# G-U-N/Phased-Consistency-Model

Measured on NVIDIA H100. Metric: distillation steps/sec (SD1.5 PCM-LoRA, bs=8/GPU), higher is better.
Workload: dtype bf16

## Files before the change

### pcm_b200/csrc/attn_wg.cu

```cuda
#include "common.cuh"
#include "wgmma.cuh"
#include "host_common.h"

namespace pcm {

namespace {

constexpr int kAwThreads = 384;
constexpr int kAwStages = 2;
constexpr int kTile = 64 * 128;

struct alignas(64) AttnWgParams {
  CUtensorMap q_map, k_map, v_map;
  bf16* out;
  float* lse;
  int H, Sq, Skv, D;
  long long ldo;
  float c;
};

template <int KB>
__global__ void __launch_bounds__(kAwThreads, 1) attn_fwd_wg_kernel(const __grid_constant__ AttnWgParams p) {
  extern __shared__ uint8_t smem_raw[];
  uint8_t* smem = reinterpret_cast<uint8_t*>((reinterpret_cast<uintptr_t>(smem_raw) + 1023) &
                                             ~static_cast<uintptr_t>(1023));
  uint8_t* sQ = smem;
  uint8_t* sK = sQ + 2 * KB * kTile;
  uint8_t* sV = sK + kAwStages * KB * kTile;
  __shared__ __align__(8) uint64_t q_bar;
  __shared__ __align__(8) uint64_t full_bar[kAwStages];
  __shared__ __align__(8) uint64_t empty_bar[kAwStages];

  const int wg = threadIdx.x >> 7;
  const int b = blockIdx.z, h = blockIdx.y, q0 = blockIdx.x * 128;
  const int nblk = (p.Skv + 63) / 64;
  constexpr uint32_t kv_bytes = 2 * KB * kTile;

  if (threadIdx.x == 0) {
    tma_prefetch_desc(&p.q_map);
    tma_prefetch_desc(&p.k_map);
    tma_prefetch_desc(&p.v_map);
    mbar_init(&q_bar, 1);
    for (int i = 0; i < kAwStages; ++i) {
      mbar_init(&full_bar[i], 1);
      mbar_init(&empty_bar[i], 2);
    }
    fence_barrier_init();
  }
  __syncthreads();
  griddep_sync();

  if (wg == 0) {
    if (threadIdx.x == 0) {
      mbar_arrive_expect_tx(&q_bar, 2 * KB * kTile);
      for (int w = 0; w < 2; ++w)
        for (int kb = 0; kb < KB; ++kb)
          tma_load_3d(sQ + (w * KB + kb) * kTile, &p.q_map, &q_bar, h * p.D + kb * 64, q0 + 64 * w, b);
      for (int j = 0; j < nblk; ++j) {
        const int st = j % kAwStages;
        mbar_wait(&empty_bar[st], ((j / kAwStages) & 1) ^ 1);
        mbar_arrive_expect_tx(&full_bar[st], kv_bytes);
        for (int kb = 0; kb < KB; ++kb) {
          tma_load_3d(sK + (st * KB + kb) * kTile, &p.k_map, &full_bar[st], h * p.D + kb * 64, j * 64, b);
          tma_load_3d(sV + (st * KB + kb) * kTile, &p.v_map, &full_bar[st], h * p.D + kb * 64, j * 64, b);
        }
      }
    }
    return;
  }

  const int cw = wg - 1, et = threadIdx.x & 127, warp = et >> 5, lane = et & 31;
  uint8_t* myQ = sQ + cw * KB * kTile;
  mbar_wait(&q_bar, 0);
  if (p.D < KB * 64) {
    const int c0 = p.D >> 3, nch = KB * 8;
    for (int i = et; i < 64 * nch; i += 128) {
      const int row = i / nch, ch = i - row * nch;
      if (ch < c0) continue;
      const uint32_t a = smem_u32(myQ + (ch >> 3) * kTile) + row * 128 + (((ch & 7) ^ (row & 7)) << 4);
      sts128(a, 0u, 0u, 0u, 0u);
    }
    fence_proxy_async();
  }
  asm volatile("bar.sync %0, 128;" ::"r"(1 + cw) : "memory");

  float o[KB][32];
#pragma unroll
  for (int kb = 0; kb < KB; ++kb)
#pragma unroll
    for (int i = 0; i < 32; ++i) o[kb][i] = 0.f;
  float m_run[2] = {-INFINITY, -INFINITY}, l_run[2] = {0.f, 0.f};
  const uint32_t q_addr = smem_u32(myQ);

  for (int j = 0; j < nblk; ++j) {
    const int st = j % kAwStages;
    mbar_wait(&full_bar[st], (j / kAwStages) & 1);
    const uint32_t k_addr = smem_u32(sK + st * KB * kTile);
    const uint32_t v_addr = smem_u32(sV + st * KB * kTile);
    float s[32];
    wgmma_fence();
#pragma unroll
    for (int kb = 0; kb < KB; ++kb)
#pragma unroll
      for (int k = 0; k < 4; ++k)
        Wgmma<64, 0, 0>::mma(s, wgmma_desc_sw128(q_addr + kb * kTile + k * 32, 16, 1024),
                             wgmma_desc_sw128(k_addr + kb * kTile + k * 32, 16, 1024), (kb | k) != 0 ? 1u : 0u);
    wgmma_commit();
    wgmma_wait<0>();
    wgmma_fence_acc(s);

    const int kbase = j * 64 + 2 * (lane & 3);
    float mx[2] = {-INFINITY, -INFINITY};
#pragma unroll
    for (int i = 0; i < 32; ++i) {
      const int key = kbase + 8 * (i >> 2) + (i & 1);
      const float v = key < p.Skv ? s[i] * p.c : -INFINITY;
      s[i] = v;
      mx[(i >> 1) & 1] = fmaxf(mx[(i >> 1) & 1], v);
    }
    float alpha[2];
#pragma unroll
    for (int r = 0; r < 2; ++r) {
      mx[r] = fmaxf(mx[r], __shfl_xor_sync(0xffffffffu, mx[r], 1));
      mx[r] = fmaxf(mx[r], __shfl_xor_sync(0xffffffffu, mx[r], 2));
      const float mn = fmaxf(m_run[r], mx[r]);
      alpha[r] = exp2f(m_run[r] - mn);
      m_run[r] = mn;
    }
    float rs[2] = {0.f, 0.f};
    uint32_t pa[4][4];
#pragma unroll
    for (int i = 0; i < 32; i += 2) {
      const int r = (i >> 1) & 1;
      const float p0 = exp2f(s[i] - m_run[r]), p1 = exp2f(s[i + 1] - m_run[r]);
      rs[r] += p0 + p1;
      pa[i >> 3][(i & 7) >> 1] = pack_bf16x2(p0, p1);
    }
#pragma unroll
    for (int r = 0; r < 2; ++r) l_run[r] = l_run[r] * alpha[r] + rs[r];
#pragma unroll
    for (int kb = 0; kb < KB; ++kb)
#pragma unroll
      for (int i = 0; i < 32; ++i) o[kb][i] *= alpha[(i >> 1) & 1];

    wgmma_fence();
#pragma unroll
    for (int kk = 0; kk < 4; ++kk)
#pragma unroll
      for (int kb = 0; kb < KB; ++kb)
        wgmma_rs_m64n64<1>(o[kb], pa[kk], wgmma_desc_sw128(v_addr + kb * kTile + kk * 2048, kTile, 1024), 1u);
    wgmma_commit();
    wgmma_wait<0>();
#pragma unroll
    for (int kb = 0; kb < KB; ++kb) wgmma_fence_acc(o[kb]);
    __syncwarp();
    if (et == 0) mbar_arrive(&empty_bar[st]);
  }

#pragma unroll
  for (int r = 0; r < 2; ++r) {
    l_run[r] += __shfl_xor_sync(0xffffffffu, l_run[r], 1);
    l_run[r] += __shfl_xor_sync(0xffffffffu, l_run[r], 2);
  }
  const int row0 = q0 + 64 * cw + 16 * warp + (lane >> 2);
#pragma unroll
  for (int r = 0; r < 2; ++r) {
    const int row = row0 + 8 * r;
    if (row >= p.Sq) continue;
    const float inv = 1.f / l_run[r];
    bf16* orow = p.out + (static_cast<long long>(b) * p.Sq + row) * p.ldo + h * p.D;
#pragma unroll
    for (int kb = 0; kb < KB; ++kb)
#pragma unroll
      for (int q = 0; q < 8; ++q) {
        const int col = kb * 64 + 8 * q + 2 * (lane & 3);
        if (col < p.D)
          *reinterpret_cast<uint32_t*>(orow + col) =
              pack_bf16x2(o[kb][4 * q + 2 * r] * inv, o[kb][4 * q + 2 * r + 1] * inv);
      }
    if ((lane & 3) == 0 && p.lse) p.lse[(static_cast<long long>(b) * p.H + h) * p.Sq + row] = m_run[r] + log2f(l_run[r]);
  }
}

struct alignas(64) AttnBwdParams {
  CUtensorMap fix0_map, fix1_map;
  CUtensorMap str0_map, str1_map;
  const float *lse, *delta;
  bf16 *out0, *out1;
  long long ld0, ld1;
  int H, Sq, Skv, D;
  int n_fix, n_str;
  float c, scale;
};

template <bool KV>
__global__ void __launch_bounds__(kAwThreads, 1) attn_bwd_wg_kernel(const __grid_constant__ AttnBwdParams p) {
  extern __shared__ uint8_t smem_raw[];
  uint8_t* smem = reinterpret_cast<uint8_t*>((reinterpret_cast<uintptr_t>(smem_raw) + 1023) &
                                             ~static_cast<uintptr_t>(1023));
  uint8_t* sF = smem;
  uint8_t* sS = sF + 4 * kTile;
  __shared__ __align__(8) uint64_t f_bar;
  __shared__ __align__(8) uint64_t full_bar[kAwStages];
  __shared__ __align__(8) uint64_t empty_bar[kAwStages];

  const int wg = threadIdx.x >> 7;
  const int b = blockIdx.z, h = blockIdx.y, r0 = blockIdx.x * 128;
  const int nblk = (p.n_str + 63) / 64;
  const int col0 = h * p.D;

  if (threadIdx.x == 0) {
    tma_prefetch_desc(&p.fix0_map);
    tma_prefetch_desc(&p.fix1_map);
    tma_prefetch_desc(&p.str0_map);
    tma_prefetch_desc(&p.str1_map);
    mbar_init(&f_bar, 1);
    for (int i = 0; i < kAwStages; ++i) {
      mbar_init(&full_bar[i], 1);
      mbar_init(&empty_bar[i], 2);
    }
    fence_barrier_init();
  }
  __syncthreads();
  griddep_sync();

  if (wg == 0) {
    regs_dealloc<40>();
    if (threadIdx.x == 0) {
      mbar_arrive_expect_tx(&f_bar, 4 * kTile);
      for (int w = 0; w < 2; ++w) {
        tma_load_3d(sF + (2 * w) * kTile, &p.fix0_map, &f_bar, col0, r0 + 64 * w, b);
        tma_load_3d(sF + (2 * w + 1) * kTile, &p.fix1_map, &f_bar, col0, r0 + 64 * w, b);
      }
      for (int j = 0; j < nblk; ++j) {
        const int st = j % kAwStages;
        mbar_wait(&empty_bar[st], ((j / kAwStages) & 1) ^ 1);
        mbar_arrive_expect_tx(&full_bar[st], 2 * kTile);
        tma_load_3d(sS + (2 * st) * kTile, &p.str0_map, &full_bar[st], col0, j * 64, b);
        tma_load_3d(sS + (2 * st + 1) * kTile, &p.str1_map, &full_bar[st], col0, j * 64, b);
      }
    }
    return;
  }

  regs_alloc<232>();
  const int cw = wg - 1, et = threadIdx.x & 127, warp = et >> 5, lane = et & 31;
  uint8_t* myF = sF + 2 * cw * kTile;
  mbar_wait(&f_bar, 0);
  if (p.D < 64) {
    const int c0 = p.D >> 3;
    for (int i = et; i < 2 * 64 * 8; i += 128) {
      const int t = i >> 9, row = (i >> 3) & 63, ch = i & 7;
      if (ch < c0) continue;
      sts128(smem_u32(myF + t * kTile) + row * 128 + ((ch ^ (row & 7)) << 4), 0u, 0u, 0u, 0u);
    }
    fence_proxy_async();
  }
  asm volatile("bar.sync %0, 128;" ::"r"(1 + cw) : "memory");

  const float* L = p.lse + (static_cast<long long>(b) * p.H + h) * p.Sq;
  const float* Dl = p.delta + (static_cast<long long>(b) * p.H + h) * p.Sq;
  const int frow = r0 + 64 * cw + 16 * warp + (lane >> 2);
  float lrow[2] = {0.f, 0.f}, drow[2] = {0.f, 0.f};
  bool rvalid[2];
#pragma unroll
  for (int r = 0; r < 2; ++r) {
    rvalid[r] = frow + 8 * r < p.n_fix;
    if (!KV) {
      lrow[r] = rvalid[r] ? L[frow + 8 * r] : INFINITY;
      drow[r] = rvalid[r] ? Dl[frow + 8 * r] : 0.f;
    }
  }
  float acc0[32], acc1[32];
#pragma unroll
  for (int i = 0; i < 32; ++i) acc0[i] = acc1[i] = 0.f;
  const uint32_t f0 = smem_u32(myF), f1 = f0 + kTile;

  for (int j = 0; j < nblk; ++j) {
    const int st = j % kAwStages;
    mbar_wait(&full_bar[st], (j / kAwStages) & 1);
    const uint32_t s0 = smem_u32(sS + 2 * st * kTile), s1 = s0 + kTile;
    float s[32], dp[32];
    wgmma_fence();
#pragma unroll
    for (int k = 0; k < 4; ++k) {
      Wgmma<64, 0, 0>::mma(s, wgmma_desc_sw128(f0 + k * 32, 16, 1024), wgmma_desc_sw128(s0 + k * 32, 16, 1024),
                           k != 0 ? 1u : 0u);
      Wgmma<64, 0, 0>::mma(dp, wgmma_desc_sw128(f1 + k * 32, 16, 1024), wgmma_desc_sw128(s1 + k * 32, 16, 1024),
                           k != 0 ? 1u : 0u);
    }
    wgmma_commit();
    float lc[16], dc[16];
    if (KV) {
#pragma unroll
      for (int q = 0; q < 8; ++q)
#pragma unroll
        for (int e = 0; e < 2; ++e) {
          const int qi = j * 64 + 8 * q + 2 * (lane & 3) + e;
          lc[2 * q + e] = qi < p.Sq ? L[qi] : INFINITY;
          dc[2 * q + e] = qi < p.Sq ? Dl[qi] : 0.f;
        }
    }
    wgmma_wait<0>();
    wgmma_fence_acc(s);
    wgmma_fence_acc(dp);
    uint32_t pa[4][4], dsa[4][4];
#pragma unroll
    for (int i = 0; i < 32; i += 2) {
      const int r = (i >> 1) & 1;
      float pv[2], g[2];
#pragma unroll
      for (int e = 0; e < 2; ++e) {
        const int col = 8 * (i >> 2) + 2 * (lane & 3) + e;
        float l, d;
        bool ok;
        if (KV) {
          l = lc[2 * (i >> 2) + e];
          d = dc[2 * (i >> 2) + e];
          ok = rvalid[r];
        } else {
          l = lrow[r];
          d = drow[r];
          ok = j * 64 + col < p.Skv;
        }
        pv[e] = ok ? exp2f(s[i + e] * p.c - l) : 0.f;
        g[e] = pv[e] * (dp[i + e] - d);
      }
      pa[i >> 3][(i & 7) >> 1] = pack_bf16x2(pv[0], pv[1]);
      dsa[i >> 3][(i & 7) >> 1] = pack_bf16x2(g[0], g[1]);
    }
    wgmma_fence();
#pragma unroll
    for (int kk = 0; kk < 4; ++kk) {
      wgmma_rs_m64n64<1>(acc0, dsa[kk], wgmma_desc_sw128(s0 + kk * 2048, kTile, 1024), 1u);
      if (KV) wgmma_rs_m64n64<1>(acc1, pa[kk], wgmma_desc_sw128(s1 + kk * 2048, kTile, 1024), 1u);
    }
    wgmma_commit();
    wgmma_wait<0>();
    wgmma_fence_acc(acc0);
    wgmma_fence_acc(acc1);
    __syncwarp();
    if (et == 0) mbar_arrive(&empty_bar[st]);
  }

#pragma unroll
  for (int r = 0; r < 2; ++r) {
    if (!rvalid[r]) continue;
    const long long row = static_cast<long long>(b) * p.n_fix + frow + 8 * r;
    bf16* o0 = p.out0 + row * p.ld0 + col0;
    bf16* o1 = KV ? p.out1 + row * p.ld1 + col0 : nullptr;
#pragma unroll
    for (int q = 0; q < 8; ++q) {
      const int col = 8 * q + 2 * (lane & 3);
      if (col < p.D) {
        *reinterpret_cast<uint32_t*>(o0 + col) =
            pack_bf16x2(acc0[4 * q + 2 * r] * p.scale, acc0[4 * q + 2 * r + 1] * p.scale);
        if (KV) *reinterpret_cast<uint32_t*>(o1 + col) = pack_bf16x2(acc1[4 * q + 2 * r], acc1[4 * q + 2 * r + 1]);
      }
    }
  }
}

int encode_seq_map(CUtensorMap* m, const void* base, int HD, int S, int B, long long ld) {
  if ((reinterpret_cast<uintptr_t>(base) & 15) != 0 || (ld & 7) != 0)
    return set_error("attention: tensor map base not 16-byte aligned or row stride not a multiple of 8");
  cuuint64_t dims[3] = {static_cast<cuuint64_t>(HD), static_cast<cuuint64_t>(S), static_cast<cuuint64_t>(B)};
  cuuint64_t strides[2] = {static_cast<cuuint64_t>(ld) * 2, static_cast<cuuint64_t>(ld) * 2 * S};
  cuuint32_t box[3] = {64, 64, 1}, estr[3] = {1, 1, 1};
  return encode_tmap(m, base, 3, dims, strides, box, estr);
}

}

int attn_fwd_wg(const void* q, const void* k, const void* v, void* out, float* lse, int B, int H, int Sq,
                int Skv, int D, long long ldq, long long ldk, long long ldv, long long ldo, float scale,
                cudaStream_t stream) {
  if (D % 8 != 0 || D > 128) return 1;
  static AttnWgParams p;
  memset(&p, 0, sizeof(p));
  int rc;
  if ((rc = encode_seq_map(&p.q_map, q, H * D, Sq, B, ldq)) != 0) return rc;
  if ((rc = encode_seq_map(&p.k_map, k, H * D, Skv, B, ldk)) != 0) return rc;
  if ((rc = encode_seq_map(&p.v_map, v, H * D, Skv, B, ldv)) != 0) return rc;
  p.out = reinterpret_cast<bf16*>(out);
  p.lse = lse;
  p.H = H; p.Sq = Sq; p.Skv = Skv; p.D = D; p.ldo = ldo;
  p.c = scale * 1.4426950408889634f;
  const dim3 grid((Sq + 127) / 128, H, B);
  if (D <= 64) {
    const size_t smem = (2 + 2 * kAwStages) * kTile + 1024;
    static bool attr = false;
    if (!attr) {
      CUDA_TRY(cudaFuncSetAttribute(attn_fwd_wg_kernel<1>, cudaFuncAttributeMaxDynamicSharedMemorySize,
                                    static_cast<int>(smem)));
      attr = true;
    }
    CUDA_TRY(launch_pdl(attn_fwd_wg_kernel<1>, grid, dim3(kAwThreads), smem, stream, p));
  } else {
    const size_t smem = 2 * (2 + 2 * kAwStages) * kTile + 1024;
    static bool attr = false;
    if (!attr) {
      CUDA_TRY(cudaFuncSetAttribute(attn_fwd_wg_kernel<2>, cudaFuncAttributeMaxDynamicSharedMemorySize,
                                    static_cast<int>(smem)));
      attr = true;
    }
    CUDA_TRY(launch_pdl(attn_fwd_wg_kernel<2>, grid, dim3(kAwThreads), smem, stream, p));
  }
  CUDA_TRY(cudaGetLastError());
  return 0;
}

int attn_bwd_wg(const void* q, const void* k, const void* v, const void* dout, const float* lse,
                const float* delta, void* dq, void* dk, void* dv, int B, int H, int Sq, int Skv, int D,
                long long ldq, long long ldk, long long ldv, long long ldo, float scale, cudaStream_t stream) {
  if (D % 8 != 0 || D > 64) return 1;
  static AttnBwdParams pk, pq;
  memset(&pk, 0, sizeof(pk));
  int rc;
  if ((rc = encode_seq_map(&pk.fix0_map, k, H * D, Skv, B, ldk)) != 0) return rc;
  if ((rc = encode_seq_map(&pk.fix1_map, v, H * D, Skv, B, ldv)) != 0) return rc;
  if ((rc = encode_seq_map(&pk.str0_map, q, H * D, Sq, B, ldq)) != 0) return rc;
  if ((rc = encode_seq_map(&pk.str1_map, dout, H * D, Sq, B, ldo)) != 0) return rc;
  pk.lse = lse; pk.delta = delta;
  pk.H = H; pk.Sq = Sq; pk.Skv = Skv; pk.D = D;
  pk.c = scale * 1.4426950408889634f;
  pq = pk;
  pk.out0 = reinterpret_cast<bf16*>(dk); pk.ld0 = ldk;
  pk.out1 = reinterpret_cast<bf16*>(dv); pk.ld1 = ldv;
  pk.n_fix = Skv; pk.n_str = Sq; pk.scale = scale;
  pq.fix0_map = pk.str0_map; pq.fix1_map = pk.str1_map;
  pq.str0_map = pk.fix0_map; pq.str1_map = pk.fix1_map;
  pq.out0 = reinterpret_cast<bf16*>(dq); pq.ld0 = ldq;
  pq.out1 = nullptr; pq.ld1 = 0;
  pq.n_fix = Sq; pq.n_str = Skv; pq.scale = scale;
  const size_t smem = (4 + 2 * kAwStages) * kTile + 1024;
  static bool attr = false;
  if (!attr) {
    CUDA_TRY(cudaFuncSetAttribute(attn_bwd_wg_kernel<true>, cudaFuncAttributeMaxDynamicSharedMemorySize,
                                  static_cast<int>(smem)));
    CUDA_TRY(cudaFuncSetAttribute(attn_bwd_wg_kernel<false>, cudaFuncAttributeMaxDynamicSharedMemorySize,
                                  static_cast<int>(smem)));
    attr = true;
  }
  CUDA_TRY(launch_pdl(attn_bwd_wg_kernel<true>, dim3((Skv + 127) / 128, H, B), dim3(kAwThreads), smem, stream, pk));
  CUDA_TRY(launch_pdl(attn_bwd_wg_kernel<false>, dim3((Sq + 127) / 128, H, B), dim3(kAwThreads), smem, stream, pq));
  CUDA_TRY(cudaGetLastError());
  return 0;
}

}
```

### pcm_b200/csrc/wgmma.cuh

```cuda
#pragma once
#include <stdint.h>

namespace pcm {

template <int N, int TA, int TB>
struct Wgmma;

template <int TA, int TB>
struct Wgmma<32, TA, TB> {
  __device__ __forceinline__ static void mma(float (&d)[16], uint64_t a, uint64_t b, uint32_t acc) {
    asm volatile(
        "{\n\t.reg .pred p;\n\t"
        "setp.ne.b32 p, %18, 0;\n\t"
        "wgmma.mma_async.sync.aligned.m64n32k16.f32.bf16.bf16 "
        "{%0, %1, %2, %3, %4, %5, %6, %7, %8, %9, %10, %11, %12, %13, %14, %15}, "
        "%16, %17, p, 1, 1, %19, %20;\n\t}"
        : "+f"(d[0]), "+f"(d[1]), "+f"(d[2]), "+f"(d[3]), "+f"(d[4]), "+f"(d[5]), "+f"(d[6]), "+f"(d[7]), "+f"(d[8]), "+f"(d[9]), "+f"(d[10]), "+f"(d[11]), "+f"(d[12]), "+f"(d[13]), "+f"(d[14]), "+f"(d[15])
        : "l"(a), "l"(b), "r"(acc), "n"(TA), "n"(TB));
  }
};

template <int TA, int TB>
struct Wgmma<64, TA, TB> {
  __device__ __forceinline__ static void mma(float (&d)[32], uint64_t a, uint64_t b, uint32_t acc) {
    asm volatile(
        "{\n\t.reg .pred p;\n\t"
        "setp.ne.b32 p, %34, 0;\n\t"
        "wgmma.mma_async.sync.aligned.m64n64k16.f32.bf16.bf16 "
        "{%0, %1, %2, %3, %4, %5, %6, %7, %8, %9, %10, %11, %12, %13, %14, %15, %16, %17, %18, %19, %20, %21, %22, %23, %24, %25, %26, %27, %28, %29, %30, %31}, "
        "%32, %33, p, 1, 1, %35, %36;\n\t}"
        : "+f"(d[0]), "+f"(d[1]), "+f"(d[2]), "+f"(d[3]), "+f"(d[4]), "+f"(d[5]), "+f"(d[6]), "+f"(d[7]), "+f"(d[8]), "+f"(d[9]), "+f"(d[10]), "+f"(d[11]), "+f"(d[12]), "+f"(d[13]), "+f"(d[14]), "+f"(d[15]), "+f"(d[16]), "+f"(d[17]), "+f"(d[18]), "+f"(d[19]), "+f"(d[20]), "+f"(d[21]), "+f"(d[22]), "+f"(d[23]), "+f"(d[24]), "+f"(d[25]), "+f"(d[26]), "+f"(d[27]), "+f"(d[28]), "+f"(d[29]), "+f"(d[30]), "+f"(d[31])
        : "l"(a), "l"(b), "r"(acc), "n"(TA), "n"(TB));
  }
};

template <int TA, int TB>
struct Wgmma<96, TA, TB> {
  __device__ __forceinline__ static void mma(float (&d)[48], uint64_t a, uint64_t b, uint32_t acc) {
    asm volatile(
        "{\n\t.reg .pred p;\n\t"
        "setp.ne.b32 p, %50, 0;\n\t"
        "wgmma.mma_async.sync.aligned.m64n96k16.f32.bf16.bf16 "
        "{%0, %1, %2, %3, %4, %5, %6, %7, %8, %9, %10, %11, %12, %13, %14, %15, %16, %17, %18, %19, %20, %21, %22, %23, %24, %25, %26, %27, %28, %29, %30, %31, %32, %33, %34, %35, %36, %37, %38, %39, %40, %41, %42, %43, %44, %45, %46, %47}, "
        "%48, %49, p, 1, 1, %51, %52;\n\t}"
        : "+f"(d[0]), "+f"(d[1]), "+f"(d[2]), "+f"(d[3]), "+f"(d[4]), "+f"(d[5]), "+f"(d[6]), "+f"(d[7]), "+f"(d[8]), "+f"(d[9]), "+f"(d[10]), "+f"(d[11]), "+f"(d[12]), "+f"(d[13]), "+f"(d[14]), "+f"(d[15]), "+f"(d[16]), "+f"(d[17]), "+f"(d[18]), "+f"(d[19]), "+f"(d[20]), "+f"(d[21]), "+f"(d[22]), "+f"(d[23]), "+f"(d[24]), "+f"(d[25]), "+f"(d[26]), "+f"(d[27]), "+f"(d[28]), "+f"(d[29]), "+f"(d[30]), "+f"(d[31]), "+f"(d[32]), "+f"(d[33]), "+f"(d[34]), "+f"(d[35]), "+f"(d[36]), "+f"(d[37]), "+f"(d[38]), "+f"(d[39]), "+f"(d[40]), "+f"(d[41]), "+f"(d[42]), "+f"(d[43]), "+f"(d[44]), "+f"(d[45]), "+f"(d[46]), "+f"(d[47])
        : "l"(a), "l"(b), "r"(acc), "n"(TA), "n"(TB));
  }
};

template <int TA, int TB>
struct Wgmma<128, TA, TB> {
  __device__ __forceinline__ static void mma(float (&d)[64], uint64_t a, uint64_t b, uint32_t acc) {
    asm volatile(
        "{\n\t.reg .pred p;\n\t"
        "setp.ne.b32 p, %66, 0;\n\t"
        "wgmma.mma_async.sync.aligned.m64n128k16.f32.bf16.bf16 "
        "{%0, %1, %2, %3, %4, %5, %6, %7, %8, %9, %10, %11, %12, %13, %14, %15, %16, %17, %18, %19, %20, %21, %22, %23, %24, %25, %26, %27, %28, %29, %30, %31, %32, %33, %34, %35, %36, %37, %38, %39, %40, %41, %42, %43, %44, %45, %46, %47, %48, %49, %50, %51, %52, %53, %54, %55, %56, %57, %58, %59, %60, %61, %62, %63}, "
        "%64, %65, p, 1, 1, %67, %68;\n\t}"
        : "+f"(d[0]), "+f"(d[1]), "+f"(d[2]), "+f"(d[3]), "+f"(d[4]), "+f"(d[5]), "+f"(d[6]), "+f"(d[7]), "+f"(d[8]), "+f"(d[9]), "+f"(d[10]), "+f"(d[11]), "+f"(d[12]), "+f"(d[13]), "+f"(d[14]), "+f"(d[15]), "+f"(d[16]), "+f"(d[17]), "+f"(d[18]), "+f"(d[19]), "+f"(d[20]), "+f"(d[21]), "+f"(d[22]), "+f"(d[23]), "+f"(d[24]), "+f"(d[25]), "+f"(d[26]), "+f"(d[27]), "+f"(d[28]), "+f"(d[29]), "+f"(d[30]), "+f"(d[31]), "+f"(d[32]), "+f"(d[33]), "+f"(d[34]), "+f"(d[35]), "+f"(d[36]), "+f"(d[37]), "+f"(d[38]), "+f"(d[39]), "+f"(d[40]), "+f"(d[41]), "+f"(d[42]), "+f"(d[43]), "+f"(d[44]), "+f"(d[45]), "+f"(d[46]), "+f"(d[47]), "+f"(d[48]), "+f"(d[49]), "+f"(d[50]), "+f"(d[51]), "+f"(d[52]), "+f"(d[53]), "+f"(d[54]), "+f"(d[55]), "+f"(d[56]), "+f"(d[57]), "+f"(d[58]), "+f"(d[59]), "+f"(d[60]), "+f"(d[61]), "+f"(d[62]), "+f"(d[63])
        : "l"(a), "l"(b), "r"(acc), "n"(TA), "n"(TB));
  }
};

template <int TA, int TB>
struct Wgmma<160, TA, TB> {
  __device__ __forceinline__ static void mma(float (&d)[80], uint64_t a, uint64_t b, uint32_t acc) {
    asm volatile(
        "{\n\t.reg .pred p;\n\t"
        "setp.ne.b32 p, %82, 0;\n\t"
        "wgmma.mma_async.sync.aligned.m64n160k16.f32.bf16.bf16 "
        "{%0, %1, %2, %3, %4, %5, %6, %7, %8, %9, %10, %11, %12, %13, %14, %15, %16, %17, %18, %19, %20, %21, %22, %23, %24, %25, %26, %27, %28, %29, %30, %31, %32, %33, %34, %35, %36, %37, %38, %39, %40, %41, %42, %43, %44, %45, %46, %47, %48, %49, %50, %51, %52, %53, %54, %55, %56, %57, %58, %59, %60, %61, %62, %63, %64, %65, %66, %67, %68, %69, %70, %71, %72, %73, %74, %75, %76, %77, %78, %79}, "
        "%80, %81, p, 1, 1, %83, %84;\n\t}"
        : "+f"(d[0]), "+f"(d[1]), "+f"(d[2]), "+f"(d[3]), "+f"(d[4]), "+f"(d[5]), "+f"(d[6]), "+f"(d[7]), "+f"(d[8]), "+f"(d[9]), "+f"(d[10]), "+f"(d[11]), "+f"(d[12]), "+f"(d[13]), "+f"(d[14]), "+f"(d[15]), "+f"(d[16]), "+f"(d[17]), "+f"(d[18]), "+f"(d[19]), "+f"(d[20]), "+f"(d[21]), "+f"(d[22]), "+f"(d[23]), "+f"(d[24]), "+f"(d[25]), "+f"(d[26]), "+f"(d[27]), "+f"(d[28]), "+f"(d[29]), "+f"(d[30]), "+f"(d[31]), "+f"(d[32]), "+f"(d[33]), "+f"(d[34]), "+f"(d[35]), "+f"(d[36]), "+f"(d[37]), "+f"(d[38]), "+f"(d[39]), "+f"(d[40]), "+f"(d[41]), "+f"(d[42]), "+f"(d[43]), "+f"(d[44]), "+f"(d[45]), "+f"(d[46]), "+f"(d[47]), "+f"(d[48]), "+f"(d[49]), "+f"(d[50]), "+f"(d[51]), "+f"(d[52]), "+f"(d[53]), "+f"(d[54]), "+f"(d[55]), "+f"(d[56]), "+f"(d[57]), "+f"(d[58]), "+f"(d[59]), "+f"(d[60]), "+f"(d[61]), "+f"(d[62]), "+f"(d[63]), "+f"(d[64]), "+f"(d[65]), "+f"(d[66]), "+f"(d[67]), "+f"(d[68]), "+f"(d[69]), "+f"(d[70]), "+f"(d[71]), "+f"(d[72]), "+f"(d[73]), "+f"(d[74]), "+f"(d[75]), "+f"(d[76]), "+f"(d[77]), "+f"(d[78]), "+f"(d[79])
        : "l"(a), "l"(b), "r"(acc), "n"(TA), "n"(TB));
  }
};

template <int TA, int TB>
struct Wgmma<192, TA, TB> {
  __device__ __forceinline__ static void mma(float (&d)[96], uint64_t a, uint64_t b, uint32_t acc) {
    asm volatile(
        "{\n\t.reg .pred p;\n\t"
        "setp.ne.b32 p, %98, 0;\n\t"
        "wgmma.mma_async.sync.aligned.m64n192k16.f32.bf16.bf16 "
        "{%0, %1, %2, %3, %4, %5, %6, %7, %8, %9, %10, %11, %12, %13, %14, %15, %16, %17, %18, %19, %20, %21, %22, %23, %24, %25, %26, %27, %28, %29, %30, %31, %32, %33, %34, %35, %36, %37, %38, %39, %40, %41, %42, %43, %44, %45, %46, %47, %48, %49, %50, %51, %52, %53, %54, %55, %56, %57, %58, %59, %60, %61, %62, %63, %64, %65, %66, %67, %68, %69, %70, %71, %72, %73, %74, %75, %76, %77, %78, %79, %80, %81, %82, %83, %84, %85, %86, %87, %88, %89, %90, %91, %92, %93, %94, %95}, "
        "%96, %97, p, 1, 1, %99, %100;\n\t}"
        : "+f"(d[0]), "+f"(d[1]), "+f"(d[2]), "+f"(d[3]), "+f"(d[4]), "+f"(d[5]), "+f"(d[6]), "+f"(d[7]), "+f"(d[8]), "+f"(d[9]), "+f"(d[10]), "+f"(d[11]), "+f"(d[12]), "+f"(d[13]), "+f"(d[14]), "+f"(d[15]), "+f"(d[16]), "+f"(d[17]), "+f"(d[18]), "+f"(d[19]), "+f"(d[20]), "+f"(d[21]), "+f"(d[22]), "+f"(d[23]), "+f"(d[24]), "+f"(d[25]), "+f"(d[26]), "+f"(d[27]), "+f"(d[28]), "+f"(d[29]), "+f"(d[30]), "+f"(d[31]), "+f"(d[32]), "+f"(d[33]), "+f"(d[34]), "+f"(d[35]), "+f"(d[36]), "+f"(d[37]), "+f"(d[38]), "+f"(d[39]), "+f"(d[40]), "+f"(d[41]), "+f"(d[42]), "+f"(d[43]), "+f"(d[44]), "+f"(d[45]), "+f"(d[46]), "+f"(d[47]), "+f"(d[48]), "+f"(d[49]), "+f"(d[50]), "+f"(d[51]), "+f"(d[52]), "+f"(d[53]), "+f"(d[54]), "+f"(d[55]), "+f"(d[56]), "+f"(d[57]), "+f"(d[58]), "+f"(d[59]), "+f"(d[60]), "+f"(d[61]), "+f"(d[62]), "+f"(d[63]), "+f"(d[64]), "+f"(d[65]), "+f"(d[66]), "+f"(d[67]), "+f"(d[68]), "+f"(d[69]), "+f"(d[70]), "+f"(d[71]), "+f"(d[72]), "+f"(d[73]), "+f"(d[74]), "+f"(d[75]), "+f"(d[76]), "+f"(d[77]), "+f"(d[78]), "+f"(d[79]), "+f"(d[80]), "+f"(d[81]), "+f"(d[82]), "+f"(d[83]), "+f"(d[84]), "+f"(d[85]), "+f"(d[86]), "+f"(d[87]), "+f"(d[88]), "+f"(d[89]), "+f"(d[90]), "+f"(d[91]), "+f"(d[92]), "+f"(d[93]), "+f"(d[94]), "+f"(d[95])
        : "l"(a), "l"(b), "r"(acc), "n"(TA), "n"(TB));
  }
};

template <int TA, int TB>
struct Wgmma<224, TA, TB> {
  __device__ __forceinline__ static void mma(float (&d)[112], uint64_t a, uint64_t b, uint32_t acc) {
    asm volatile(
        "{\n\t.reg .pred p;\n\t"
        "setp.ne.b32 p, %114, 0;\n\t"
        "wgmma.mma_async.sync.aligned.m64n224k16.f32.bf16.bf16 "
        "{%0, %1, %2, %3, %4, %5, %6, %7, %8, %9, %10, %11, %12, %13, %14, %15, %16, %17, %18, %19, %20, %21, %22, %23, %24, %25, %26, %27, %28, %29, %30, %31, %32, %33, %34, %35, %36, %37, %38, %39, %40, %41, %42, %43, %44, %45, %46, %47, %48, %49, %50, %51, %52, %53, %54, %55, %56, %57, %58, %59, %60, %61, %62, %63, %64, %65, %66, %67, %68, %69, %70, %71, %72, %73, %74, %75, %76, %77, %78, %79, %80, %81, %82, %83, %84, %85, %86, %87, %88, %89, %90, %91, %92, %93, %94, %95, %96, %97, %98, %99, %100, %101, %102, %103, %104, %105, %106, %107, %108, %109, %110, %111}, "
        "%112, %113, p, 1, 1, %115, %116;\n\t}"
        : "+f"(d[0]), "+f"(d[1]), "+f"(d[2]), "+f"(d[3]), "+f"(d[4]), "+f"(d[5]), "+f"(d[6]), "+f"(d[7]), "+f"(d[8]), "+f"(d[9]), "+f"(d[10]), "+f"(d[11]), "+f"(d[12]), "+f"(d[13]), "+f"(d[14]), "+f"(d[15]), "+f"(d[16]), "+f"(d[17]), "+f"(d[18]), "+f"(d[19]), "+f"(d[20]), "+f"(d[21]), "+f"(d[22]), "+f"(d[23]), "+f"(d[24]), "+f"(d[25]), "+f"(d[26]), "+f"(d[27]), "+f"(d[28]), "+f"(d[29]), "+f"(d[30]), "+f"(d[31]), "+f"(d[32]), "+f"(d[33]), "+f"(d[34]), "+f"(d[35]), "+f"(d[36]), "+f"(d[37]), "+f"(d[38]), "+f"(d[39]), "+f"(d[40]), "+f"(d[41]), "+f"(d[42]), "+f"(d[43]), "+f"(d[44]), "+f"(d[45]), "+f"(d[46]), "+f"(d[47]), "+f"(d[48]), "+f"(d[49]), "+f"(d[50]), "+f"(d[51]), "+f"(d[52]), "+f"(d[53]), "+f"(d[54]), "+f"(d[55]), "+f"(d[56]), "+f"(d[57]), "+f"(d[58]), "+f"(d[59]), "+f"(d[60]), "+f"(d[61]), "+f"(d[62]), "+f"(d[63]), "+f"(d[64]), "+f"(d[65]), "+f"(d[66]), "+f"(d[67]), "+f"(d[68]), "+f"(d[69]), "+f"(d[70]), "+f"(d[71]), "+f"(d[72]), "+f"(d[73]), "+f"(d[74]), "+f"(d[75]), "+f"(d[76]), "+f"(d[77]), "+f"(d[78]), "+f"(d[79]), "+f"(d[80]), "+f"(d[81]), "+f"(d[82]), "+f"(d[83]), "+f"(d[84]), "+f"(d[85]), "+f"(d[86]), "+f"(d[87]), "+f"(d[88]), "+f"(d[89]), "+f"(d[90]), "+f"(d[91]), "+f"(d[92]), "+f"(d[93]), "+f"(d[94]), "+f"(d[95]), "+f"(d[96]), "+f"(d[97]), "+f"(d[98]), "+f"(d[99]), "+f"(d[100]), "+f"(d[101]), "+f"(d[102]), "+f"(d[103]), "+f"(d[104]), "+f"(d[105]), "+f"(d[106]), "+f"(d[107]), "+f"(d[108]), "+f"(d[109]), "+f"(d[110]), "+f"(d[111])
        : "l"(a), "l"(b), "r"(acc), "n"(TA), "n"(TB));
  }
};

template <int TA, int TB>
struct Wgmma<256, TA, TB> {
  __device__ __forceinline__ static void mma(float (&d)[128], uint64_t a, uint64_t b, uint32_t acc) {
    asm volatile(
        "{\n\t.reg .pred p;\n\t"
        "setp.ne.b32 p, %130, 0;\n\t"
        "wgmma.mma_async.sync.aligned.m64n256k16.f32.bf16.bf16 "
        "{%0, %1, %2, %3, %4, %5, %6, %7, %8, %9, %10, %11, %12, %13, %14, %15, %16, %17, %18, %19, %20, %21, %22, %23, %24, %25, %26, %27, %28, %29, %30, %31, %32, %33, %34, %35, %36, %37, %38, %39, %40, %41, %42, %43, %44, %45, %46, %47, %48, %49, %50, %51, %52, %53, %54, %55, %56, %57, %58, %59, %60, %61, %62, %63, %64, %65, %66, %67, %68, %69, %70, %71, %72, %73, %74, %75, %76, %77, %78, %79, %80, %81, %82, %83, %84, %85, %86, %87, %88, %89, %90, %91, %92, %93, %94, %95, %96, %97, %98, %99, %100, %101, %102, %103, %104, %105, %106, %107, %108, %109, %110, %111, %112, %113, %114, %115, %116, %117, %118, %119, %120, %121, %122, %123, %124, %125, %126, %127}, "
        "%128, %129, p, 1, 1, %131, %132;\n\t}"
        : "+f"(d[0]), "+f"(d[1]), "+f"(d[2]), "+f"(d[3]), "+f"(d[4]), "+f"(d[5]), "+f"(d[6]), "+f"(d[7]), "+f"(d[8]), "+f"(d[9]), "+f"(d[10]), "+f"(d[11]), "+f"(d[12]), "+f"(d[13]), "+f"(d[14]), "+f"(d[15]), "+f"(d[16]), "+f"(d[17]), "+f"(d[18]), "+f"(d[19]), "+f"(d[20]), "+f"(d[21]), "+f"(d[22]), "+f"(d[23]), "+f"(d[24]), "+f"(d[25]), "+f"(d[26]), "+f"(d[27]), "+f"(d[28]), "+f"(d[29]), "+f"(d[30]), "+f"(d[31]), "+f"(d[32]), "+f"(d[33]), "+f"(d[34]), "+f"(d[35]), "+f"(d[36]), "+f"(d[37]), "+f"(d[38]), "+f"(d[39]), "+f"(d[40]), "+f"(d[41]), "+f"(d[42]), "+f"(d[43]), "+f"(d[44]), "+f"(d[45]), "+f"(d[46]), "+f"(d[47]), "+f"(d[48]), "+f"(d[49]), "+f"(d[50]), "+f"(d[51]), "+f"(d[52]), "+f"(d[53]), "+f"(d[54]), "+f"(d[55]), "+f"(d[56]), "+f"(d[57]), "+f"(d[58]), "+f"(d[59]), "+f"(d[60]), "+f"(d[61]), "+f"(d[62]), "+f"(d[63]), "+f"(d[64]), "+f"(d[65]), "+f"(d[66]), "+f"(d[67]), "+f"(d[68]), "+f"(d[69]), "+f"(d[70]), "+f"(d[71]), "+f"(d[72]), "+f"(d[73]), "+f"(d[74]), "+f"(d[75]), "+f"(d[76]), "+f"(d[77]), "+f"(d[78]), "+f"(d[79]), "+f"(d[80]), "+f"(d[81]), "+f"(d[82]), "+f"(d[83]), "+f"(d[84]), "+f"(d[85]), "+f"(d[86]), "+f"(d[87]), "+f"(d[88]), "+f"(d[89]), "+f"(d[90]), "+f"(d[91]), "+f"(d[92]), "+f"(d[93]), "+f"(d[94]), "+f"(d[95]), "+f"(d[96]), "+f"(d[97]), "+f"(d[98]), "+f"(d[99]), "+f"(d[100]), "+f"(d[101]), "+f"(d[102]), "+f"(d[103]), "+f"(d[104]), "+f"(d[105]), "+f"(d[106]), "+f"(d[107]), "+f"(d[108]), "+f"(d[109]), "+f"(d[110]), "+f"(d[111]), "+f"(d[112]), "+f"(d[113]), "+f"(d[114]), "+f"(d[115]), "+f"(d[116]), "+f"(d[117]), "+f"(d[118]), "+f"(d[119]), "+f"(d[120]), "+f"(d[121]), "+f"(d[122]), "+f"(d[123]), "+f"(d[124]), "+f"(d[125]), "+f"(d[126]), "+f"(d[127])
        : "l"(a), "l"(b), "r"(acc), "n"(TA), "n"(TB));
  }
};

template <int TB>
__device__ __forceinline__ void wgmma_rs_m64n64(float (&d)[32], const uint32_t (&a)[4], uint64_t b, uint32_t acc) {
  asm volatile(
      "{\n\t.reg .pred p;\n\t"
      "setp.ne.b32 p, %37, 0;\n\t"
      "wgmma.mma_async.sync.aligned.m64n64k16.f32.bf16.bf16 "
      "{%0, %1, %2, %3, %4, %5, %6, %7, %8, %9, %10, %11, %12, %13, %14, %15, %16, %17, %18, %19, %20, %21, %22, %23, %24, %25, %26, %27, %28, %29, %30, %31}, "
      "{%32, %33, %34, %35}, %36, p, 1, 1, %38;\n\t}"
      : "+f"(d[0]), "+f"(d[1]), "+f"(d[2]), "+f"(d[3]), "+f"(d[4]), "+f"(d[5]), "+f"(d[6]), "+f"(d[7]), "+f"(d[8]), "+f"(d[9]), "+f"(d[10]), "+f"(d[11]), "+f"(d[12]), "+f"(d[13]), "+f"(d[14]), "+f"(d[15]), "+f"(d[16]), "+f"(d[17]), "+f"(d[18]), "+f"(d[19]), "+f"(d[20]), "+f"(d[21]), "+f"(d[22]), "+f"(d[23]), "+f"(d[24]), "+f"(d[25]), "+f"(d[26]), "+f"(d[27]), "+f"(d[28]), "+f"(d[29]), "+f"(d[30]), "+f"(d[31])
      : "r"(a[0]), "r"(a[1]), "r"(a[2]), "r"(a[3]), "l"(b), "r"(acc), "n"(TB));
}

}
```

Before: 7.895.

## Software-pipeline attention backward wgmma and trim head-dim and K-step work

Restructures the attention backward kernel so the S/dP wgmmas of block j overlap with the dS·K / P·dO accumulation wgmmas of block j-1. The smem ring is deepened from two to three stages. LSE/delta stats for the KV kernel are loaded once per block into shared memory instead of per-lane gathers from global memory. Templates on head dim so D=40 (SD1.5 heads) uses m64n40 wgmmas and skips the unused K-steps, and masking only runs on the final ragged block. This adds register pressure from the extra live operands and more shared memory, which may hurt occupancy or cause spills.

```diff
diff --git a/pcm_b200/csrc/attn_wg.cu b/pcm_b200/csrc/attn_wg.cu
--- a/pcm_b200/csrc/attn_wg.cu
+++ b/pcm_b200/csrc/attn_wg.cu
@@ -8,6 +8,7 @@
 
 constexpr int kAwThreads = 384;
 constexpr int kAwStages = 2;
+constexpr int kBwdStages = 3;
 constexpr int kTile = 64 * 128;
 
 struct alignas(64) AttnWgParams {
@@ -18,6 +19,18 @@
   long long ldo;
   float c;
 };
+
+__device__ __forceinline__ void keep_operand(uint32_t (&a)[4][4]) {
+#pragma unroll
+  for (int i = 0; i < 4; ++i)
+#pragma unroll
+    for (int k = 0; k < 4; ++k) asm volatile("" : "+r"(a[i][k])::"memory");
+}
+
+__device__ __forceinline__ void pack_operand(uint32_t (&a)[4][4], const float (&x)[32]) {
+#pragma unroll
+  for (int i = 0; i < 32; i += 2) a[i >> 3][(i & 7) >> 1] = pack_bf16x2(x[i], x[i + 1]);
+}
 
 template <int KB>
 __global__ void __launch_bounds__(kAwThreads, 1) attn_fwd_wg_kernel(const __grid_constant__ AttnWgParams p) {
@@ -148,7 +161,7 @@
     for (int kk = 0; kk < 4; ++kk)
 #pragma unroll
       for (int kb = 0; kb < KB; ++kb)
-        wgmma_rs_m64n64<1>(o[kb], pa[kk], wgmma_desc_sw128(v_addr + kb * kTile + kk * 2048, kTile, 1024), 1u);
+        WgmmaRs<64, 1>::mma(o[kb], pa[kk], wgmma_desc_sw128(v_addr + kb * kTile + kk * 2048, kTile, 1024), 1u);
     wgmma_commit();
     wgmma_wait<0>();
 #pragma unroll
@@ -193,16 +206,47 @@
   float c, scale;
 };
 
-template <bool KV>
+template <bool KV, bool MASK>
+__device__ __forceinline__ void bwd_elementwise(float (&s)[32], float (&dp)[32], const float (&lc)[16],
+                                                const float (&dc)[16], const float (&lrow)[2],
+                                                const float (&drow)[2], const bool (&rvalid)[2], float c,
+                                                int kcol, int Skv) {
+#pragma unroll
+  for (int i = 0; i < 32; i += 2) {
+    const int r = (i >> 1) & 1;
+#pragma unroll
+    for (int e = 0; e < 2; ++e) {
+      float l, d;
+      bool ok;
+      if (KV) {
+        l = lc[2 * (i >> 2) + e];
+        d = dc[2 * (i >> 2) + e];
+        ok = rvalid[r];
+      } else {
+        l = lrow[r];
+        d = drow[r];
+        ok = !MASK || kcol + 8 * (i >> 2) + e < Skv;
+      }
+      const float pv = ok ? exp2f(s[i + e] * c - l) : 0.f;
+      s[i + e] = pv;
+      dp[i + e] = pv * (dp[i + e] - d);
+    }
+  }
+}
+
+template <bool KV, int NV>
 __global__ void __launch_bounds__(kAwThreads, 1) attn_bwd_wg_kernel(const __grid_constant__ AttnBwdParams p) {
+  constexpr int kStages = kBwdStages;
+  constexpr int KS = (NV + 15) / 16;
   extern __shared__ uint8_t smem_raw[];
   uint8_t* smem = reinterpret_cast<uint8_t*>((reinterpret_cast<uintptr_t>(smem_raw) + 1023) &
                                              ~static_cast<uintptr_t>(1023));
   uint8_t* sF = smem;
   uint8_t* sS = sF + 4 * kTile;
   __shared__ __align__(8) uint64_t f_bar;
-  __shared__ __align__(8) uint64_t full_bar[kAwStages];
-  __shared__ __align__(8) uint64_t empty_bar[kAwStages];
+  __shared__ __align__(8) uint64_t full_bar[kStages];
+  __shared__ __align__(8) uint64_t empty_bar[kStages];
+  __shared__ float stats[2][2][2][64];
 
   const int wg = threadIdx.x >> 7;
   const int b = blockIdx.z, h = blockIdx.y, r0 = blockIdx.x * 128;
@@ -215,7 +259,7 @@
     tma_prefetch_desc(&p.str0_map);
     tma_prefetch_desc(&p.str1_map);
     mbar_init(&f_bar, 1);
-    for (int i = 0; i < kAwStages; ++i) {
+    for (int i = 0; i < kStages; ++i) {
       mbar_init(&full_bar[i], 1);
       mbar_init(&empty_bar[i], 2);
     }
@@ -233,8 +277,8 @@
         tma_load_3d(sF + (2 * w + 1) * kTile, &p.fix1_map, &f_bar, col0, r0 + 64 * w, b);
       }
       for (int j = 0; j < nblk; ++j) {
-        const int st = j % kAwStages;
-        mbar_wait(&empty_bar[st], ((j / kAwStages) & 1) ^ 1);
+        const int st = j % kStages;
+        mbar_wait(&empty_bar[st], ((j / kStages) & 1) ^ 1);
         mbar_arrive_expect_tx(&full_bar[st], 2 * kTile);
         tma_load_3d(sS + (2 * st) * kTile, &p.str0_map, &full_bar[st], col0, j * 64, b);
         tma_load_3d(sS + (2 * st + 1) * kTile, &p.str1_map, &full_bar[st], col0, j * 64, b);
@@ -271,77 +315,105 @@
       drow[r] = rvalid[r] ? Dl[frow + 8 * r] : 0.f;
     }
   }
-  float acc0[32], acc1[32];
-#pragma unroll
-  for (int i = 0; i < 32; ++i) acc0[i] = acc1[i] = 0.f;
+  float acc0[NV / 2], acc1[NV / 2];
+#pragma unroll
+  for (int i = 0; i < NV / 2; ++i) acc0[i] = acc1[i] = 0.f;
   const uint32_t f0 = smem_u32(myF), f1 = f0 + kTile;
-
-  for (int j = 0; j < nblk; ++j) {
-    const int st = j % kAwStages;
-    mbar_wait(&full_bar[st], (j / kAwStages) & 1);
+  const bool ragged = !KV && (p.Skv & 63) != 0;
+  float s[32], dp[32];
+  uint32_t pa[4][4], dsa[4][4];
+
+  auto issue_sdp = [&](int st) {
     const uint32_t s0 = smem_u32(sS + 2 * st * kTile), s1 = s0 + kTile;
-    float s[32], dp[32];
-    wgmma_fence();
-#pragma unroll
-    for (int k = 0; k < 4; ++k) {
-      Wgmma<64, 0, 0>::mma(s, wgmma_desc_sw128(f0 + k * 32, 16, 1024), wgmma_desc_sw128(s0 + k * 32, 16, 1024),
-                           k != 0 ? 1u : 0u);
-      Wgmma<64, 0, 0>::mma(dp, wgmma_desc_sw128(f1 + k * 32, 16, 1024), wgmma_desc_sw128(s1 + k * 32, 16, 1024),
-                           k != 0 ? 1u : 0u);
+    Wgmma<64, 0, 0>::mma_first(s, wgmma_desc_sw128(f0, 16, 1024), wgmma_desc_sw128(s0, 16, 1024));
+    Wgmma<64, 0, 0>::mma_first(dp, wgmma_desc_sw128(f1, 16, 1024), wgmma_desc_sw128(s1, 16, 1024));
+#pragma unroll
+    for (int k = 1; k < KS; ++k) {
+      Wgmma<64, 0, 0>::mma(s, wgmma_desc_sw128(f0 + k * 32, 16, 1024), wgmma_desc_sw128(s0 + k * 32, 16, 1024), 1u);
+      Wgmma<64, 0, 0>::mma(dp, wgmma_desc_sw128(f1 + k * 32, 16, 1024), wgmma_desc_sw128(s1 + k * 32, 16, 1024), 1u);
     }
     wgmma_commit();
+  };
+  auto issue_acc = [&](int st) {
+    const uint32_t s0 = smem_u32(sS + 2 * st * kTile), s1 = s0 + kTile;
+#pragma unroll
+    for (int kk = 0; kk < 4; ++kk) {
+      WgmmaRs<NV, 1>::mma(acc0, dsa[kk], wgmma_desc_sw128(s0 + kk * 2048, kTile, 1024), 1u);
+      if (KV) WgmmaRs<NV, 1>::mma(acc1, pa[kk], wgmma_desc_sw128(s1 + kk * 2048, kTile, 1024), 1u);
+    }
+    wgmma_commit();
+  };
+  auto load_stat = [&](int j) {
+    const int qi = j * 64 + (et & 63);
+    if (et < 64) return qi < p.Sq ? L[qi] : INFINITY;
+    return qi < p.Sq ? Dl[qi] : 0.f;
+  };
+  auto publish_stat = [&](int j, float v) {
+    stats[cw][j & 1][et >> 6][et & 63] = v;
+    asm volatile("bar.sync %0, 128;" ::"r"(1 + cw) : "memory");
+  };
+  auto elementwise = [&](int j) {
+    const int kcol = j * 64 + 2 * (lane & 3);
     float lc[16], dc[16];
     if (KV) {
 #pragma unroll
-      for (int q = 0; q < 8; ++q)
-#pragma unroll
-        for (int e = 0; e < 2; ++e) {
-          const int qi = j * 64 + 8 * q + 2 * (lane & 3) + e;
-          lc[2 * q + e] = qi < p.Sq ? L[qi] : INFINITY;
-          dc[2 * q + e] = qi < p.Sq ? Dl[qi] : 0.f;
-        }
-    }
-    wgmma_wait<0>();
+      for (int q = 0; q < 8; ++q) {
+        const float2 l2 = *reinterpret_cast<const float2*>(&stats[cw][j & 1][0][8 * q + 2 * (lane & 3)]);
+        const float2 d2 = *reinterpret_cast<const float2*>(&stats[cw][j & 1][1][8 * q + 2 * (lane & 3)]);
+        lc[2 * q] = l2.x;
+        lc[2 * q + 1] = l2.y;
+        dc[2 * q] = d2.x;
+        dc[2 * q + 1] = d2.y;
+      }
+    }
+    if (ragged && j == nblk - 1)
+      bwd_elementwise<KV, true>(s, dp, lc, dc, lrow, drow, rvalid, p.c, kcol, p.Skv);
+    else
+      bwd_elementwise<KV, false>(s, dp, lc, dc, lrow, drow, rvalid, p.c, kcol, p.Skv);
+  };
+
+  if (KV) publish_stat(0, load_stat(0));
+  mbar_wait(&full_bar[0], 0);
+  wgmma_fence();
+  issue_sdp(0);
+  float nxt = KV ? load_stat(1) : 0.f;
+  wgmma_wait<0>();
+  wgmma_fence_acc(s);
+  wgmma_fence_acc(dp);
+  elementwise(0);
+  if (KV) publish_stat(1, nxt);
+  pack_operand(pa, s);
+  pack_operand(dsa, dp);
+
+  for (int j = 1; j < nblk; ++j) {
+    const int st = j % kStages, pst = (j - 1) % kStages;
+    mbar_wait(&full_bar[st], (j / kStages) & 1);
+    wgmma_fence();
+    issue_sdp(st);
+    issue_acc(pst);
+    if (KV) nxt = load_stat(j + 1);
+    wgmma_wait<1>();
     wgmma_fence_acc(s);
     wgmma_fence_acc(dp);
-    uint32_t pa[4][4], dsa[4][4];
-#pragma unroll
-    for (int i = 0; i < 32; i += 2) {
-      const int r = (i >> 1) & 1;
-      float pv[2], g[2];
-#pragma unroll
-      for (int e = 0; e < 2; ++e) {
-        const int col = 8 * (i >> 2) + 2 * (lane & 3) + e;
-        float l, d;
-        bool ok;
-        if (KV) {
-          l = lc[2 * (i >> 2) + e];
-          d = dc[2 * (i >> 2) + e];
-          ok = rvalid[r];
-        } else {
-          l = lrow[r];
-          d = drow[r];
-          ok = j * 64 + col < p.Skv;
-        }
-        pv[e] = ok ? exp2f(s[i + e] * p.c - l) : 0.f;
-        g[e] = pv[e] * (dp[i + e] - d);
-      }
-      pa[i >> 3][(i & 7) >> 1] = pack_bf16x2(pv[0], pv[1]);
-      dsa[i >> 3][(i & 7) >> 1] = pack_bf16x2(g[0], g[1]);
-    }
-    wgmma_fence();
-#pragma unroll
-    for (int kk = 0; kk < 4; ++kk) {
-      wgmma_rs_m64n64<1>(acc0, dsa[kk], wgmma_desc_sw128(s0 + kk * 2048, kTile, 1024), 1u);
-      if (KV) wgmma_rs_m64n64<1>(acc1, pa[kk], wgmma_desc_sw128(s1 + kk * 2048, kTile, 1024), 1u);
-    }
-    wgmma_commit();
+    elementwise(j);
+    if (KV) publish_stat(j + 1, nxt);
     wgmma_wait<0>();
     wgmma_fence_acc(acc0);
     wgmma_fence_acc(acc1);
+    keep_operand(pa);
+    keep_operand(dsa);
     __syncwarp();
-    if (et == 0) mbar_arrive(&empty_bar[st]);
-  }
+    if (et == 0) mbar_arrive(&empty_bar[pst]);
+    pack_operand(pa, s);
+    pack_operand(dsa, dp);
+  }
+  wgmma_fence();
+  issue_acc((nblk - 1) % kStages);
+  wgmma_wait<0>();
+  wgmma_fence_acc(acc0);
+  wgmma_fence_acc(acc1);
+  keep_operand(pa);
+  keep_operand(dsa);
 
 #pragma unroll
   for (int r = 0; r < 2; ++r) {
@@ -350,7 +422,7 @@
     bf16* o0 = p.out0 + row * p.ld0 + col0;
     bf16* o1 = KV ? p.out1 + row * p.ld1 + col0 : nullptr;
 #pragma unroll
-    for (int q = 0; q < 8; ++q) {
+    for (int q = 0; q < NV / 8; ++q) {
       const int col = 8 * q + 2 * (lane & 3);
       if (col < p.D) {
         *reinterpret_cast<uint32_t*>(o0 + col) =
@@ -368,6 +440,19 @@
   cuuint64_t strides[2] = {static_cast<cuuint64_t>(ld) * 2, static_cast<cuuint64_t>(ld) * 2 * S};
   cuuint32_t box[3] = {64, 64, 1}, estr[3] = {1, 1, 1};
   return encode_tmap(m, base, 3, dims, strides, box, estr);
+}
+
+template <bool KV, int NV>
+cudaError_t launch_bwd(dim3 grid, cudaStream_t stream, const AttnBwdParams& p) {
+  const size_t smem = (4 + 2 * kBwdStages) * kTile + 1024;
+  static bool attr = false;
+  if (!attr) {
+    const cudaError_t e = cudaFuncSetAttribute(attn_bwd_wg_kernel<KV, NV>, cudaFuncAttributeMaxDynamicSharedMemorySize,
+                                               static_cast<int>(smem));
+    if (e != cudaSuccess) return e;
+    attr = true;
+  }
+  return launch_pdl(attn_bwd_wg_kernel<KV, NV>, grid, dim3(kAwThreads), smem, stream, p);
 }
 
 }
@@ -433,17 +518,14 @@
   pq.out0 = reinterpret_cast<bf16*>(dq); pq.ld0 = ldq;
   pq.out1 = nullptr; pq.ld1 = 0;
   pq.n_fix = Sq; pq.n_str = Skv; pq.scale = scale;
-  const size_t smem = (4 + 2 * kAwStages) * kTile + 1024;
-  static bool attr = false;
-  if (!attr) {
-    CUDA_TRY(cudaFuncSetAttribute(attn_bwd_wg_kernel<true>, cudaFuncAttributeMaxDynamicSharedMemorySize,
-                                  static_cast<int>(smem)));
-    CUDA_TRY(cudaFuncSetAttribute(attn_bwd_wg_kernel<false>, cudaFuncAttributeMaxDynamicSharedMemorySize,
-                                  static_cast<int>(smem)));
-    attr = true;
-  }
-  CUDA_TRY(launch_pdl(attn_bwd_wg_kernel<true>, dim3((Skv + 127) / 128, H, B), dim3(kAwThreads), smem, stream, pk));
-  CUDA_TRY(launch_pdl(attn_bwd_wg_kernel<false>, dim3((Sq + 127) / 128, H, B), dim3(kAwThreads), smem, stream, pq));
+  const dim3 gk((Skv + 127) / 128, H, B), gq((Sq + 127) / 128, H, B);
+  if (D <= 40) {
+    CUDA_TRY((launch_bwd<true, 40>)(gk, stream, pk));
+    CUDA_TRY((launch_bwd<false, 40>)(gq, stream, pq));
+  } else {
+    CUDA_TRY((launch_bwd<true, 64>)(gk, stream, pk));
+    CUDA_TRY((launch_bwd<false, 64>)(gq, stream, pq));
+  }
   CUDA_TRY(cudaGetLastError());
   return 0;
 }
diff --git a/pcm_b200/csrc/wgmma.cuh b/pcm_b200/csrc/wgmma.cuh
--- a/pcm_b200/csrc/wgmma.cuh
+++ b/pcm_b200/csrc/wgmma.cuh
@@ -31,6 +31,14 @@
         "%32, %33, p, 1, 1, %35, %36;\n\t}"
         : "+f"(d[0]), "+f"(d[1]), "+f"(d[2]), "+f"(d[3]), "+f"(d[4]), "+f"(d[5]), "+f"(d[6]), "+f"(d[7]), "+f"(d[8]), "+f"(d[9]), "+f"(d[10]), "+f"(d[11]), "+f"(d[12]), "+f"(d[13]), "+f"(d[14]), "+f"(d[15]), "+f"(d[16]), "+f"(d[17]), "+f"(d[18]), "+f"(d[19]), "+f"(d[20]), "+f"(d[21]), "+f"(d[22]), "+f"(d[23]), "+f"(d[24]), "+f"(d[25]), "+f"(d[26]), "+f"(d[27]), "+f"(d[28]), "+f"(d[29]), "+f"(d[30]), "+f"(d[31])
         : "l"(a), "l"(b), "r"(acc), "n"(TA), "n"(TB));
+  }
+  __device__ __forceinline__ static void mma_first(float (&d)[32], uint64_t a, uint64_t b) {
+    asm volatile(
+        "wgmma.mma_async.sync.aligned.m64n64k16.f32.bf16.bf16 "
+        "{%0, %1, %2, %3, %4, %5, %6, %7, %8, %9, %10, %11, %12, %13, %14, %15, %16, %17, %18, %19, %20, %21, %22, %23, %24, %25, %26, %27, %28, %29, %30, %31}, "
+        "%32, %33, 0, 1, 1, %34, %35;"
+        : "=f"(d[0]), "=f"(d[1]), "=f"(d[2]), "=f"(d[3]), "=f"(d[4]), "=f"(d[5]), "=f"(d[6]), "=f"(d[7]), "=f"(d[8]), "=f"(d[9]), "=f"(d[10]), "=f"(d[11]), "=f"(d[12]), "=f"(d[13]), "=f"(d[14]), "=f"(d[15]), "=f"(d[16]), "=f"(d[17]), "=f"(d[18]), "=f"(d[19]), "=f"(d[20]), "=f"(d[21]), "=f"(d[22]), "=f"(d[23]), "=f"(d[24]), "=f"(d[25]), "=f"(d[26]), "=f"(d[27]), "=f"(d[28]), "=f"(d[29]), "=f"(d[30]), "=f"(d[31])
+        : "l"(a), "l"(b), "n"(TA), "n"(TB));
   }
 };
 
@@ -118,16 +126,35 @@
   }
 };
 
+template <int N, int TB>
+struct WgmmaRs;
+
 template <int TB>
-__device__ __forceinline__ void wgmma_rs_m64n64(float (&d)[32], const uint32_t (&a)[4], uint64_t b, uint32_t acc) {
-  asm volatile(
-      "{\n\t.reg .pred p;\n\t"
-      "setp.ne.b32 p, %37, 0;\n\t"
-      "wgmma.mma_async.sync.aligned.m64n64k16.f32.bf16.bf16 "
-      "{%0, %1, %2, %3, %4, %5, %6, %7, %8, %9, %10, %11, %12, %13, %14, %15, %16, %17, %18, %19, %20, %21, %22, %23, %24, %25, %26, %27, %28, %29, %30, %31}, "
-      "{%32, %33, %34, %35}, %36, p, 1, 1, %38;\n\t}"
-      : "+f"(d[0]), "+f"(d[1]), "+f"(d[2]), "+f"(d[3]), "+f"(d[4]), "+f"(d[5]), "+f"(d[6]), "+f"(d[7]), "+f"(d[8]), "+f"(d[9]), "+f"(d[10]), "+f"(d[11]), "+f"(d[12]), "+f"(d[13]), "+f"(d[14]), "+f"(d[15]), "+f"(d[16]), "+f"(d[17]), "+f"(d[18]), "+f"(d[19]), "+f"(d[20]), "+f"(d[21]), "+f"(d[22]), "+f"(d[23]), "+f"(d[24]), "+f"(d[25]), "+f"(d[26]), "+f"(d[27]), "+f"(d[28]), "+f"(d[29]), "+f"(d[30]), "+f"(d[31])
-      : "r"(a[0]), "r"(a[1]), "r"(a[2]), "r"(a[3]), "l"(b), "r"(acc), "n"(TB));
-}
+struct WgmmaRs<40, TB> {
+  __device__ __forceinline__ static void mma(float (&d)[20], const uint32_t (&a)[4], uint64_t b, uint32_t acc) {
+    asm volatile(
+        "{\n\t.reg .pred p;\n\t"
+        "setp.ne.b32 p, %25, 0;\n\t"
+        "wgmma.mma_async.sync.aligned.m64n40k16.f32.bf16.bf16 "
+        "{%0, %1, %2, %3, %4, %5, %6, %7, %8, %9, %10, %11, %12, %13, %14, %15, %16, %17, %18, %19}, "
+        "{%20, %21, %22, %23}, %24, p, 1, 1, %26;\n\t}"
+        : "+f"(d[0]), "+f"(d[1]), "+f"(d[2]), "+f"(d[3]), "+f"(d[4]), "+f"(d[5]), "+f"(d[6]), "+f"(d[7]), "+f"(d[8]), "+f"(d[9]), "+f"(d[10]), "+f"(d[11]), "+f"(d[12]), "+f"(d[13]), "+f"(d[14]), "+f"(d[15]), "+f"(d[16]), "+f"(d[17]), "+f"(d[18]), "+f"(d[19])
+        : "r"(a[0]), "r"(a[1]), "r"(a[2]), "r"(a[3]), "l"(b), "r"(acc), "n"(TB));
+  }
+};
+
+template <int TB>
+struct WgmmaRs<64, TB> {
+  __device__ __forceinline__ static void mma(float (&d)[32], const uint32_t (&a)[4], uint64_t b, uint32_t acc) {
+    asm volatile(
+        "{\n\t.reg .pred p;\n\t"
+        "setp.ne.b32 p, %37, 0;\n\t"
+        "wgmma.mma_async.sync.aligned.m64n64k16.f32.bf16.bf16 "
+        "{%0, %1, %2, %3, %4, %5, %6, %7, %8, %9, %10, %11, %12, %13, %14, %15, %16, %17, %18, %19, %20, %21, %22, %23, %24, %25, %26, %27, %28, %29, %30, %31}, "
+        "{%32, %33, %34, %35}, %36, p, 1, 1, %38;\n\t}"
+        : "+f"(d[0]), "+f"(d[1]), "+f"(d[2]), "+f"(d[3]), "+f"(d[4]), "+f"(d[5]), "+f"(d[6]), "+f"(d[7]), "+f"(d[8]), "+f"(d[9]), "+f"(d[10]), "+f"(d[11]), "+f"(d[12]), "+f"(d[13]), "+f"(d[14]), "+f"(d[15]), "+f"(d[16]), "+f"(d[17]), "+f"(d[18]), "+f"(d[19]), "+f"(d[20]), "+f"(d[21]), "+f"(d[22]), "+f"(d[23]), "+f"(d[24]), "+f"(d[25]), "+f"(d[26]), "+f"(d[27]), "+f"(d[28]), "+f"(d[29]), "+f"(d[30]), "+f"(d[31])
+        : "r"(a[0]), "r"(a[1]), "r"(a[2]), "r"(a[3]), "l"(b), "r"(acc), "n"(TB));
+  }
+};
 
 }
```

After: 8.155 (median of 6 runs). +3.3%, better.
